# Franc-Z/CuClarabel

Hardware: AMD Instinct MI355X
Metric: KKT factorize+solve/sec (fp64) per IPM iter, 100k-var SOCP (higher is better)
Workload: dtype f64

## Files before the change

### cuclarabel_amd/csrc/factor_kernels.hip

```cpp
#include "kernels.hpp"
#include "knobs.hpp"
#include <utility>

namespace hipkkt {

__device__ inline double rl_f64(double v, int lane)
{
    const int lo = __builtin_amdgcn_readlane(__double2loint(v), lane);
    const int hi = __builtin_amdgcn_readlane(__double2hiint(v), lane);
    return __hiloint2double(hi, lo);
}
#define WAVE_FENCE() asm volatile("" ::: "memory")

__device__ __forceinline__ void lds_add(double* p, double v)
{
    __hip_atomic_fetch_add(p, v, __ATOMIC_RELAXED, __HIP_MEMORY_SCOPE_WORKGROUP);
}
#define OV_LD(p) __hip_atomic_load((p), __ATOMIC_RELAXED, __HIP_MEMORY_SCOPE_AGENT)
#define OV_ST(p, v) __hip_atomic_store((p), (v), __ATOMIC_RELAXED, __HIP_MEMORY_SCOPE_AGENT)
__device__ inline bool ov_wait_ge(const int* counter, int target, int* abort_word, long long t0, long long limit, int who = 0, int info = 0,
                                  int* seen_min = nullptr)
{
    for (;;) {
        const int seen = __hip_atomic_load(counter, __ATOMIC_RELAXED, __HIP_MEMORY_SCOPE_AGENT);
// ... 577 lines not shown
        }
        if (A.stamps) { long long t1 = wall_clock64(); t_iii += t1 - t0; }
    }
    __syncthreads();
    HIPKKT_STAMP(A, 4);
    if (!OV) for (int idx = tid; idx < f * nc; idx += BS) {
        const int j = idx / f, r = idx - j * f;
        if (!SLICED) {
            if (r >= j) F[idx] = P[r + pcol(j, f)];
        } else if (r >= nc) {
            F[(r_lo + r - nc) + (int64_t)j * ff] = P[r + pcol(j, f)];
        } else if (first && r >= j) {
            F[r + (int64_t)j * ff] = P[r + pcol(j, f)];
        }
    }
    __syncthreads();
    HIPKKT_STAMP(A, 5);
    if (A.stamps && blockIdx.x == 0 && tid == 0) {
        A.stamps[A.stamp_row * 16 + 8] = t_i;
        A.stamps[A.stamp_row * 16 + 9] = t_ii;
        A.stamps[A.stamp_row * 16 + 10] = t_iii;
        A.stamps[A.stamp_row * 16 + 11] = f;
        A.stamps[A.stamp_row * 16 + 12] = nc;
        A.stamps[A.stamp_row * 16 + 13] = T.child_ptr[s + 1] - T.child_ptr[s];
        A.stamps[A.stamp_row * 16 + 14] = clock64() - clk0;
    }
}

constexpr int TS = 64;
constexpr int KC = 16;

constexpr int LDA = TS + 16;

template <bool OV, bool PIPE>
__global__ __launch_bounds__(256) __attribute__((amdgpu_waves_per_eu(OV ? 3 : 4))) void k_schur(FactorArgs A, const int2* __restrict__ tiles, int tile_begin, int ntiles)
{
    __shared__ __attribute__((aligned(16))) double smem_s[TS * (TS + 1) + (OV ? 2 * KC * LDA + 2 : 0)];
    double (*As)[LDA] = reinterpret_cast<double (*)[LDA]>(smem_s + (OV ? TS * (TS + 1) : 0));
    double (*Bs)[LDA] = reinterpret_cast<double (*)[LDA]>(smem_s + (OV ? TS * (TS + 1) : 0) + KC * LDA);
    double (*Ct)[TS + 1] = reinterpret_cast<double (*)[TS + 1]>(smem_s);
    volatile int* sh_ok = reinterpret_cast<volatile int*>(smem_s + TS * (TS + 1) + 2 * KC * LDA);
    static_assert(2 * KC * LDA <= TS * (TS + 1), "operand chunks must fit under the tile buffer");
    const int tid = threadIdx.x, lane = tid & 63;
    const int wv = __builtin_amdgcn_readfirstlane(tid >> 6);
    const TreeDev& T = A.T;
    for (int tix = blockIdx.x; tix < ntiles; tix += gridDim.x) {
    const int2 tl = tiles[tile_begin + tix];
    const int s = tl.x;
    const int ti = tl.y >> 16, tj = tl.y & 0xffff;
    const int c0 = T.sn_start[s];
    const int nc = T.sn_start[s + 1] - c0;
    const int nb = (int)(T.rowptr[s + 1] - T.rowptr[s]);
    const int f = nc + nb;
    const double* __restrict__ F = A.fronts + T.front_off[s];
    double* __restrict__ U = A.upd + T.upd_off[s];
    const int r0 = ti * TS, q0 = tj * TS;
    const int nr = min(TS, nb - r0), nq = min(TS, nb - q0);

    const int wr = wv >> 1, wc = wv & 1;
    const bool active = !(ti == tj && wr < wc) && 32 * wr < nr && 32 * wc < nq;
    d4_t acc[2][2];
#pragma unroll
    for (int i = 0; i < 2; ++i)
#pragma unroll
        for (int j = 0; j < 2; ++j) acc[i][j] = (d4_t){0.0, 0.0, 0.0, 0.0};
    const int ml = lane & 15, mk = lane >> 4;
    const int64_t* __restrict__ tc = T.tile_cut + 5 * (int64_t)(tile_begin + tix);
    const int64_t i0 = tc[wv], i1 = tc[wv + 1];
    static_assert(sizeof(SubItem) == 16, "SubItem is read as an int4");
    const int4* __restrict__ sit4 = reinterpret_cast<const int4*>(T.sitems);
    int4 mine = (i0 < i1) ? sit4[min(i0 + lane, i1 - 1)] : make_int4(0, 0, 0, 0);
    auto pass_through = [&]() {
        constexpr int PT = 16;
        const int rlo = nc + r0;
        double* ct = &Ct[0][0];
        for (int64_t base = i0; base < i1; base += 64) {
            if (base > i0) mine = sit4[min(base + lane, i1 - 1)];
            const int n = (int)min((int64_t)64, i1 - base);
            for (int z0 = 0; z0 < n; z0 += PT) {
                double v[PT];
                int tg[PT];
#pragma unroll
                for (int z = 0; z < PT; ++z) {
                    const int src = min(z0 + z, 63);
                    const unsigned lo = (unsigned)__builtin_amdgcn_readlane(mine.x, src);
                    const int hi = __builtin_amdgcn_readlane(mine.y, src);
                    const int relstart = __builtin_amdgcn_readlane(mine.z, src);
                    const int cq = __builtin_amdgcn_readlane(mine.w, src);
                    const int64_t uoff = ((int64_t)hi << 32) | lo;
                    const int cnt = (z0 + z < n) ? (cq & 0xff) : 0, qcol = (cq >> 8) & 0xff;
                    const bool ok = lane < cnt;
                    v[z] = ok ? A.upd[uoff + lane] : 0.0;
                    tg[z] = ok ? qcol * (TS + 1) + (T.rel[relstart + lane] - rlo) : -1;
                }
#pragma unroll
                for (int z = 0; z < PT; ++z) if (tg[z] >= 0) lds_add(ct + tg[z], v[z]);
            }
        }
    };
    const int64_t dense_off_s = T.dense_off[s];
    auto dense_ptr = [&]() -> const double* {
        return dense_off_s >= 0 ? A.upd + dense_off_s + (int64_t)(nc + r0) + (int64_t)(nc + q0) * f : nullptr;
    };
    if (OV) {
        const double* __restrict__ Ud = dense_ptr();
        auto dense_at = [&](int a, int b) -> double {
            return (Ud && a < nr && b < nq && (r0 + a) >= (q0 + b)) ? Ud[a + (int64_t)b * f] : 0.0;
        };
// ... 176 lines not shown
void launch_front_wave(const FactorArgs& a, int begin, int count, int slice_doubles, hipStream_t st)
{
    if (count <= 0) return;
    init_factor_lds();
    hipLaunchKernelGGL(k_front_wave, dim3((count + 3) / 4), dim3(256), (size_t)4 * slice_doubles * sizeof(double), st,
                       a, begin, count, slice_doubles);
}
void launch_panel(const FactorArgs& a, int begin, int count, int bs, size_t lds, hipStream_t st)
{
    if (count <= 0) return;
    init_factor_lds();
    if (a.ov) {
        if (bs == 1024) hipLaunchKernelGGL((k_panel<1024, false, true>), dim3(count), dim3(1024), lds, st, a, begin);
        else if (bs == 512) hipLaunchKernelGGL((k_panel<512, false, true>), dim3(count), dim3(512), lds, st, a, begin);
        else hipLaunchKernelGGL((k_panel<256, false, true>), dim3(count), dim3(256), lds, st, a, begin);
        return;
    }
    if (bs == 1024) hipLaunchKernelGGL((k_panel<1024, false, false>), dim3(count), dim3(1024), lds, st, a, begin);
    else if (bs == 512) hipLaunchKernelGGL((k_panel<512, false, false>), dim3(count), dim3(512), lds, st, a, begin);
    else hipLaunchKernelGGL((k_panel<256, false, false>), dim3(count), dim3(256), lds, st, a, begin);
}
void launch_panel_sliced(const FactorArgs& a, int begin, int count, size_t lds, hipStream_t st)
{
    if (count <= 0) return;
    init_factor_lds();
    if (a.ov) hipLaunchKernelGGL((k_panel<1024, true, true>), dim3(count), dim3(1024), lds, st, a, begin);
    else hipLaunchKernelGGL((k_panel<1024, true, false>), dim3(count), dim3(1024), lds, st, a, begin);
}
void launch_schur(const FactorArgs& a, const int2* tiles, int tile_begin, int ntiles, hipStream_t st, int ov_grid, int tile_nc)
{
    if (ntiles <= 0) return;
    const int pipe_tiles = knobs().schur_pipe_tiles;
    const int pipe_nc = knobs().schur_pipe_nc;
    if (a.ov) hipLaunchKernelGGL((k_schur<true, true>), dim3(std::max(1, std::min(ntiles, ov_grid))), dim3(256), 0, st, a, tiles, tile_begin, ntiles);
    else if (ntiles > pipe_tiles && tile_nc >= pipe_nc) hipLaunchKernelGGL((k_schur<false, true>), dim3(ntiles), dim3(256), 0, st, a, tiles, tile_begin, ntiles);
    else hipLaunchKernelGGL((k_schur<false, false>), dim3(ntiles), dim3(256), 0, st, a, tiles, tile_begin, ntiles);
}

template <int VARIANT>
__global__ __launch_bounds__(256) void k_handover_litmus(double* payload, int* sig, int* ack, int words, int rounds,
                                                         unsigned long long* mismatches, unsigned long long* timeouts)
{
    __shared__ int sh_ok;
    const int pair = blockIdx.x >> 1, tid = threadIdx.x;
    const bool producer = (blockIdx.x & 1) == 0;
    double* pl = payload + (size_t)pair * words;
    const long long limit = 20000000;
    unsigned long long bad = 0;
    for (int r = 1; r <= rounds; ++r) {
        const long long t0 = wall_clock64();
        if (tid == 0) sh_ok = 1;
        __syncthreads();
        if (producer) {
            for (int w = tid; w < words; w += 256) {
                const double v = (double)r * 1024.0 + (double)w;
                if (VARIANT == 2) pl[w] = v; else OV_ST(pl + w, v);
            }
            if (VARIANT != 1) asm volatile("s_waitcnt vmcnt(0)" ::: "memory");
            __syncthreads();
            if (tid == 0) {
                OV_ST(sig + pair, r);
                for (;;) {
                    if (OV_LD(ack + pair) >= r) break;
                    if (wall_clock64() - t0 > limit) { sh_ok = 0; atomicAdd(timeouts, 1ull); break; }
                    __builtin_amdgcn_s_sleep(1);
                }
            }
            __syncthreads();
            if (!sh_ok) return;
// ... 31 lines not shown
```

### cuclarabel_amd/csrc/hipkkt.hip

```cpp
#include "../../include/hipkkt.h"

#include <hip/hip_runtime.h>

#include <algorithm>
#include <cfloat>
#include <chrono>
#include <cmath>
#include <cstdio>
#include <cstdlib>
#include <cstring>
#include <array>
#include <functional>
#include <map>
#include <memory>
#include <mutex>
#include <stdexcept>
#include <string>
#include <vector>

#include "kernels.hpp"
#include "kkt_assembly.hpp"
#include "symbolic.hpp"
#include "knobs.hpp"
#include "schedule.hpp"
#include "iterate_rows.hpp"

namespace hipkkt {

static thread_local std::string g_last_error;

struct ArgError : std::runtime_error { using std::runtime_error::runtime_error; };

#define HIP_CHECK(expr)                                                                          \
    do {                                                                                         \
        hipError_t e_ = (expr);                                                                  \
        if (e_ != hipSuccess)                                                                    \
            throw HipError(std::string(#expr) + ": " + hipGetErrorString(e_));                   \
    } while (0)

template <class T>
struct DBuf {
    T* p = nullptr;
    size_t n = 0;
    DBuf() = default;
    DBuf(const DBuf&) = delete;
    DBuf& operator=(const DBuf&) = delete;
    ~DBuf() { if (p) (void)hipFree(p); }
    void alloc(size_t count)
    {
        if (p) { (void)hipFree(p); p = nullptr; }
        n = count;
        HIP_CHECK(hipMalloc((void**)&p, std::max<size_t>(count, 1) * sizeof(T)));
    }
    void zero(hipStream_t st) { HIP_CHECK(hipMemsetAsync(p, 0, std::max<size_t>(n, 1) * sizeof(T), st)); }
    template <class V>
    void upload(const std::vector<V>& v)
    {
// ... 951 lines not shown
    {
        return knobs().factor_overlap;
    }
    bool ov_active() const { return overlap_wanted() && !ov_disabled && sch.ov_first < sch.launches.size(); }

    int* flags_ptr() { return flags.p; }

private:
    DBuf<int> d_sn_start, d_rows, d_rel, d_ncolpar, d_child_ptr, d_child_idx, d_ksrc, d_kdst, d_sched, d_perm;
    DBuf<int64_t> d_rowptr, d_front_off, d_upd_off, d_kptr;
    DBuf<signed char> d_psign;
    DBuf<double> fronts, upd, Dinv, xp, uvec, tinv;
    DBuf<double> xp_m, uvec_m;
    DBuf<int> d_iperm;
    size_t multi_cap = 0;
    DBuf<int64_t> d_tinv_off;
    DBuf<double> top_stamps;
    int n_stamp_sweeps = 0;
#ifdef HIPKKT_EXPERIMENTS
    int n_skipw_calls = 0;
#endif
    DBuf<int> d_tinv_list;
    DBuf<int> flags;
    DBuf<int64_t> stamps;
    DBuf<int64_t> d_tiles;
    DBuf<int64_t> d_cut_ptr;
    DBuf<int> d_cuts;
    DBuf<int64_t> d_item_ptr;
    DBuf<int64_t> d_items;
    DBuf<int64_t> d_dense_off;
    DBuf<int64_t> d_wave_cut;
    DBuf<int64_t> d_sitems;
    DBuf<int64_t> d_tile_cut;
    DBuf<int64_t> d_desc;
    DBuf<int64_t> d_sdesc;
    std::vector<int64_t> slice_kptr;
    std::vector<int> slice_nk;
    DBuf<int> d_spos, d_sn_parent, top_flags;
    DBuf<int> d_tk_pos, d_tk_sl, d_tbase;
    DBuf<double> xf;
    bool ov_disabled = false;
    bool ov_concurrent = false;
    DBuf<int> d_ov_prog, d_ov_done, d_ov_ntiles, d_ov_sprog, d_ov_sbase, d_ov_started;
    hipStream_t ov_stream = nullptr;
    hipEvent_t ev_ov_fork = nullptr, ev_ov_join = nullptr, ev_dev_done = nullptr;
    bool ov_join_pending = false;
    size_t nr_cap = 1;
    int top_epoch = 0;
    DBuf<int> d_gl_src, d_udst;
    DBuf<int64_t> d_glm_ptr, d_hp_lidx, d_pr_ptr;
    DBuf<int> d_udst_m, d_hp_col, d_hp_row, d_pr_slot;
    int n_pull_rows = 0;
    Schedule sch;
    DeviceLimits dev;
    NrGrids top_grid_nr;

    TreeDev tree() const
    {
        TreeDev t;
        t.nsuper = S.nsuper;
        t.sn_start = d_sn_start.p; t.rowptr = d_rowptr.p; t.rows = d_rows.p; t.rel = d_rel.p;
        t.ncolpar = d_ncolpar.p; t.front_off = d_front_off.p; t.upd_off = d_upd_off.p;
        t.child_ptr = d_child_ptr.p; t.child_idx = d_child_idx.p; t.kptr = d_kptr.p;
        t.ksrc = d_ksrc.p; t.kdst = d_kdst.p; t.sched = d_sched.p; t.psign = d_psign.p; t.perm = d_perm.p;
        t.dense_off = d_dense_off.p; t.item_ptr = d_item_ptr.p; t.items = (const ExtItem*)d_items.p; t.gl_ptr = d_item_ptr.p; t.gl_src = d_gl_src.p; t.udst = d_udst.p;
        t.glm_ptr = d_glm_ptr.p; t.udst_m = d_udst_m.p; t.hp_col = d_hp_col.p; t.hp_row = d_hp_row.p; t.hp_lidx = d_hp_lidx.p; t.pr_ptr = d_pr_ptr.p; t.pr_slot = d_pr_slot.p;
        t.cut_ptr = d_cut_ptr.p; t.cuts = d_cuts.p; t.wave_cut = d_wave_cut.p; t.tinv_off = d_tinv_off.p;
        t.sitems = (const SubItem*)d_sitems.p; t.tile_cut = d_tile_cut.p; t.desc = (const FrontDesc*)d_desc.p; t.sdesc = (const FrontDesc*)d_sdesc.p;
        t.spos = d_spos.p; t.sn_parent = d_sn_parent.p;
        return t;
    }

    int front_size(int s) const { return hipkkt::front_size(S, s); }

    void build_records(const std::vector<int64_t>& glptr, const std::vector<int>& gsrc)
    {
        if (sch.rec_refused_bytes && knobs().verbose)
            std::fprintf(stderr, "[hipkkt] packed sweep records would take %.0f MB: legacy layout\n", sch.rec_refused_bytes / 1048576.0);
        const int64_t total = sch.rec_bytes;
        if (total <= 0) return;
        std::vector<int64_t> store((size_t)(total / 8) + 8, 0);
        char* base = reinterpret_cast<char*>(store.data());
        for (size_t q = 0; q < sch.launches.size(); ++q) {
            const Launch& L = sch.launches[q];
            const bool leaf = rec_no_slots(sch.launches, q);
            RecClass classes[2];
            const int nclasses = rec_classes(L, classes);
            for (int ci = 0; ci < nclasses; ++ci) {
                const RecClass& c = classes[ci];
                const int fmax = L.rec.fmax[c.cls];
                for (int k = 0; k < c.count; ++k) {
                    const int sn = sch.sched[(size_t)(c.first + k)];
                    char* rec = base + L.rec.off[c.cls] + (int64_t)k * L.rec.stride[c.cls];
                    const int nc = S.sn_start[sn + 1] - S.sn_start[sn], nb = (int)(S.rowptr[sn + 1] - S.rowptr[sn]), f = nc + nb;
                    if (f > fmax) throw std::runtime_error("packed record: front larger than its class");
                    SolveHdr h{};
                    h.mat_off = c.cls == 0 ? h_toff[(size_t)sn] : S.front_off[sn];
                    h.rp = S.rowptr[sn];
                    h.s = sn; h.c0 = S.sn_start[sn]; h.nc = nc; h.nb = nb;
                    h.par = S.sn_parent[sn];
                    h.nchild = sch.nch.empty() ? 0 : sch.nch[(size_t)sn];
// ... 202 lines not shown
            std::vector<int> gsrc((size_t)ptr[nloc]);
            {
                std::vector<int64_t> nxt(ptr.begin(), ptr.end() - 1);
                for (int p = 0; p < S.nsuper; ++p)
                    for (int e = S.child_ptr[p]; e < S.child_ptr[p + 1]; ++e) {
                        int c = S.child_idx[e];
                        for (int64_t q = S.rowptr[c]; q < S.rowptr[c + 1]; ++q) gsrc[nxt[lbase(p) + S.rel[q]]++] = (int)q;
                    }
            }
            if (S.rows.size() >= ((size_t)1 << 31)) throw std::runtime_error("row structure exceeds int32 indexing");
            if (knobs().verbose >= 2 && sch.top_launches > 0) {
                long hist[6] = {0, 0, 0, 0, 0, 0};
                long fronts_over8 = 0, fronts_over12 = 0, nf = 0;
                int64_t gmax = 0;
                for (size_t q = sch.launches.size() - sch.top_launches; q < sch.launches.size(); ++q)
                    for (int t = sch.launches[q].begin; t < sch.launches[q].begin + sch.launches[q].count; ++t) {
                        const int sn = sch.sched[(size_t)t];
                        const int f = front_size(sn);
                        int64_t fm = 0;
                        for (int i = 0; i < f; ++i) {
                            const int64_t n = ptr[lbase(sn) + i + 1] - ptr[lbase(sn) + i];
                            hist[n == 0 ? 0 : n <= 4 ? 1 : n <= 8 ? 2 : n <= 12 ? 3 : n <= 16 ? 4 : 5]++;
                            fm = std::max(fm, n);
                        }
                        gmax = std::max(gmax, fm);
                        fronts_over8 += fm > 8; fronts_over12 += fm > 12; ++nf;
                    }
                std::fprintf(stderr, "[hipkkt] persistent solve set: gather sources per row: 0: %ld, 1-4: %ld, 5-8: %ld, 9-12: %ld, "
                             "13-16: %ld, more: %ld (max %lld); fronts with a row over 8: %ld, over 12: %ld of %ld\n",
                             hist[0], hist[1], hist[2], hist[3], hist[4], hist[5], (long long)gmax, fronts_over8, fronts_over12, nf);
            }
            d_item_ptr.upload(ptr);
            static_assert(sizeof(ExtItem) == 32, "ExtItem layout");
            std::vector<int> dense_child((size_t)S.nsuper, -1);
            std::vector<int64_t> dense_off((size_t)S.nsuper, -1);
            const bool dense_on = knobs().dense_child;
            int64_t n_dense = 0;
            for (int p = 0; dense_on && p < S.nsuper; ++p) {
                if (sch.tile_base[p] < 0) continue;
                const int fp = front_size(p);
                for (int e = S.child_ptr[p]; e < S.child_ptr[p + 1]; ++e) {
                    const int c = S.child_idx[e];
                    const int nbc = (int)(S.rowptr[c + 1] - S.rowptr[c]);
                    if (nbc != fp) continue;
                    bool ident = true;
                    for (int q = 0; ident && q < nbc; ++q) ident = S.rel[S.rowptr[c] + q] == q;
                    if (!ident) continue;
                    dense_child[(size_t)p] = c;
                    dense_off[(size_t)p] = S.upd_off[c];
                    ++n_dense;
                    break;
                }
            }
            d_dense_off.upload(dense_off);
            if (knobs().verbose) std::fprintf(stderr, "[hipkkt] dense children: %lld\n", (long long)n_dense);
            std::vector<int64_t> pptr((size_t)S.N + 1, 0);
            for (int c = 0; c < S.nsuper; ++c) {
                int p = S.sn_parent[c];
                if (p < 0 || dense_child[(size_t)p] == c) continue;
                const int pnc = S.sn_start[p + 1] - S.sn_start[p];
                const int nbc = (int)(S.rowptr[c + 1] - S.rowptr[c]);
                for (int b = 0; b < nbc; ++b) {
                    const int r = S.rel[S.rowptr[c] + b];
                    if (r >= pnc) break;
                    pptr[(size_t)S.sn_start[p] + r + 1] += (nbc - b + 63) / 64;
                }
            }
            for (int i = 0; i < S.N; ++i) pptr[i + 1] += pptr[i];
            std::vector<ExtItem> items((size_t)pptr[S.N]);
            {
                std::vector<int64_t> nxt(pptr.begin(), pptr.end() - 1);
                for (int p = 0; p < S.nsuper; ++p) {
                    const int pnc = S.sn_start[p + 1] - S.sn_start[p];
                    for (int e = S.child_ptr[p]; e < S.child_ptr[p + 1]; ++e) {
                        int c = S.child_idx[e];
                        if (dense_child[(size_t)p] == c) continue;
                        int nbc = (int)(S.rowptr[c + 1] - S.rowptr[c]);
                        for (int b = 0; b < nbc; ++b) {
                            int64_t q = S.rowptr[c] + b;
                            const int r = S.rel[q];
                            if (r >= pnc) break;
                            for (int a = b; a < nbc; a += 64) {
                                ExtItem it;
                                it.uoff = S.upd_off[c] + (int64_t)b * nbc + a;
                                it.relstart = (int)(S.rowptr[c] + a);
                                it.cnt = std::min(64, nbc - a);
// ... 34 lines not shown
                        if (e.rfirst >= nc && (e.rlast < r_lo || e.rfirst >= r_lo + rs)) continue;
                        items.push_back(e);
                    }
                }
                scp[(size_t)nc] = (int64_t)items.size();
                const int64_t I0 = scp[0], I1 = scp[(size_t)nc];
                int j = 0;
                int64_t* w = wcut.data() + ((size_t)S.nsuper + q) * 17;
                for (int k = 0; k < 16; ++k) {
                    const int64_t target = I0 + ((I1 - I0) * k) / 16;
                    while (j < nc && scp[(size_t)j] < target) ++j;
                    w[k] = scp[(size_t)j];
                }
                w[16] = I1;
            }
            std::vector<int64_t> raw(std::max<size_t>(items.size(), 1) * 4);
            std::memcpy(raw.data(), items.data(), items.size() * sizeof(ExtItem));
            d_items.upload(raw);
            d_wave_cut.upload(wcut);
            if (knobs().verbose) {
                if (knobs().verbose >= 2) {
                    for (size_t q = sch.sched.size() > 12 ? sch.sched.size() - 12 : 0; q < sch.sched.size(); ++q) {
                        const int sn = sch.sched[q];
                        const int64_t* w = wcut.data() + (size_t)sn * 17;
                        int64_t mx = 0, rows = 0;
                        for (int k = 0; k < 16; ++k) mx = std::max(mx, w[k + 1] - w[k]);
                        for (int64_t it = w[0]; it < w[16]; ++it) rows += items[(size_t)it].cnt;
                        std::fprintf(stderr, "[hipkkt] front %d f %d nc %d kids %d: %lld panel items (%lld entries), largest wave slice %lld\n",
                                     sn, front_size(sn), S.sn_start[sn + 1] - S.sn_start[sn], S.child_ptr[sn + 1] - S.child_ptr[sn],
                                     (long long)(w[16] - w[0]), (long long)rows, (long long)mx);
                    }
                }
            }
            static_assert(sizeof(SubItem) == 16, "SubItem layout");
            const int64_t ntile = (int64_t)sch.tiles.size();
            std::vector<int64_t> cnt((size_t)ntile * 64 + 1, 0);
            auto for_each_sub = [&](auto&& fn) {
                for (int p = 0; p < S.nsuper; ++p) {
                    if (sch.tile_base[p] < 0) continue;
                    const int pnc = S.sn_start[p + 1] - S.sn_start[p];
                    for (int e = S.child_ptr[p]; e < S.child_ptr[p + 1]; ++e) {
                        const int c = S.child_idx[e];
                        if (dense_child[(size_t)p] == c) continue;
                        const int nbc = (int)(S.rowptr[c + 1] - S.rowptr[c]);
                        const int* rl = S.rel.data() + S.rowptr[c];
                        for (int b = 0; b < nbc; ++b) {
                            if (rl[b] < pnc) continue;
                            const int j = rl[b] - pnc, tj = j >> 6;
                            int a = b;
                            while (a < nbc) {
                                const int ti = (rl[a] - pnc) >> 6;
                                int a2 = a;
                                while (a2 < nbc && ((rl[a2] - pnc) >> 6) == ti) ++a2;
                                const int64_t tile = sch.tile_base[p] + (int64_t)ti * (ti + 1) / 2 + tj;
                                fn(tile, j & 63, c, b, a, a2 - a, nbc);
                                a = a2;
                            }
                        }
                    }
                }
            };
            for_each_sub([&](int64_t tile, int q, int, int, int, int, int) { cnt[tile * 64 + q + 1]++; });
            for (size_t i = 0; i + 1 < cnt.size(); ++i) cnt[i + 1] += cnt[i];
            std::vector<SubItem> sit((size_t)cnt.back());
            {
                std::vector<int64_t> nx(cnt.begin(), cnt.end() - 1);
                for_each_sub([&](int64_t tile, int q, int c, int b, int a, int n, int nbc) {
                    SubItem si;
                    si.uoff = S.upd_off[c] + (int64_t)b * nbc + a;
                    si.relstart = (int)(S.rowptr[c] + a);
                    si.cnt = (unsigned char)n;
                    si.qcol = (unsigned char)q;
                    si.pad = 0;
                    sit[(size_t)nx[tile * 64 + q]++] = si;
                });
            }
            std::vector<int64_t> tcut((size_t)ntile * 5 + 5, 0);
            for (int64_t t = 0; t < ntile; ++t) {
                const int64_t* cp = cnt.data() + t * 64;
                const int64_t I0 = cp[0], I1 = cp[64];
                int q = 0;
                for (int w = 0; w < 4; ++w) {
                    const int64_t target = I0 + ((I1 - I0) * w) / 4;
                    while (q < 64 && cp[q] < target) ++q;
                    tcut[t * 5 + w] = cp[q];
                }
                tcut[t * 5 + 4] = I1;
            }
            std::vector<int64_t> tiles_up(sch.tiles);
            {
                const int tile_xcd = knobs().tile_xcd;
                if (tile_xcd > 0) {
                    std::vector<int64_t> nc2(tcut);
                    for (const Launch& L : sch.launches) {
                        if (L.small || L.count < tile_xcd || L.ntiles <= 0) continue;
                        std::vector<std::pair<int64_t, int64_t>> rng;
                        for (int t = L.begin; t < L.begin + L.count; ++t) {
                            const int sn = sch.sched[(size_t)t];
                            if (sch.tile_base[sn] < 0) continue;
                            const int nb = front_size(sn) - (S.sn_start[sn + 1] - S.sn_start[sn]);
                            const int k = (nb + 63) / 64;
                            if (k > 0) rng.push_back({sch.tile_base[sn], sch.tile_base[sn] + (int64_t)k * (k + 1) / 2});
                        }
                        int64_t pos = L.tile_begin;
                        for (size_t g0 = 0; g0 < rng.size(); g0 += 8) {
                            const size_t g1 = std::min(rng.size(), g0 + 8);
                            int64_t longest = 0;
                            for (size_t x = g0; x < g1; ++x) longest = std::max(longest, rng[x].second - rng[x].first);
                            for (int64_t j = 0; j < longest; ++j)
                                for (size_t x = g0; x < g1; ++x)
                                    if (rng[x].first + j < rng[x].second) {
                                        const int64_t from = rng[x].first + j;
                                        tiles_up[(size_t)pos] = sch.tiles[(size_t)from];
                                        for (int w = 0; w < 5; ++w) nc2[(size_t)pos * 5 + w] = tcut[(size_t)from * 5 + w];
                                        ++pos;
                                    }
                        }
                        if (pos != (int64_t)L.tile_begin + L.ntiles) throw std::runtime_error("tile permutation lost a tile");
                    }
                    tcut.swap(nc2);
                }
            }
            d_tiles.upload(tiles_up);
            std::vector<int64_t> raw2(sit.size() * 2);
            std::memcpy(raw2.data(), sit.data(), sit.size() * sizeof(SubItem));
            d_sitems.upload(raw2);
            d_tile_cut.upload(tcut);
            d_gl_src.upload(gsrc);
            build_records(ptr, gsrc);
            std::vector<int> ud(std::max<size_t>(S.rows.size(), 1), 0);
            for (size_t g = 0; g < gsrc.size(); ++g) ud[(size_t)gsrc[g]] = (int)g;
            d_udst.upload(ud);
            {
                std::vector<int> row_sn(std::max<size_t>(S.rows.size(), 1), -1);
                for (int c = 0; c < S.nsuper; ++c)
                    for (int64_t q = S.rowptr[c]; q < S.rowptr[c + 1]; ++q) row_sn[(size_t)q] = c;
                std::vector<int64_t> mptr((size_t)nloc + 1, 0), prp(1, 0);
                std::vector<int> udm(std::max<size_t>(S.rows.size(), 1), -1), hcol, prs;
                std::vector<int64_t> hl;
                int64_t slot = 0;
                for (int64_t lc = 0; lc < nloc; ++lc) {
                    mptr[(size_t)lc] = slot;
                    bool any = false;
                    for (int64_t g = ptr[(size_t)lc]; g < ptr[(size_t)lc + 1] && !any; ++g) any = pulled[(size_t)row_sn[(size_t)gsrc[(size_t)g]]] != 0;
                    if (any) prs.push_back((int)slot++);
                    for (int64_t g = ptr[(size_t)lc]; g < ptr[(size_t)lc + 1]; ++g) {
                        const int q = gsrc[(size_t)g], c = row_sn[(size_t)q];
                        if (pulled[(size_t)c]) {
                            hcol.push_back(S.sn_start[c]);
                            hl.push_back(S.front_off[c] + 1 + ((int64_t)q - S.rowptr[c]));
                        } else {
                            udm[(size_t)q] = (int)slot++;
                        }
                    }
                    if (any) prp.push_back((int64_t)hcol.size());
                }
                mptr[(size_t)nloc] = slot;
                n_pull_rows = (int)prs.size();
                if (hcol.empty()) { hcol.push_back(0); hl.push_back(0); }
                if (prs.empty()) prs.push_back(0);
// ... 2566 lines not shown
```

### cuclarabel_amd/csrc/kernels.hpp

```cpp
#pragma once
#include <hip/hip_runtime.h>
#include "launch_shapes.hpp"
#include <cstdint>
#include <mutex>
#include <stdexcept>
#include <string>

namespace hipkkt {

struct HipError : std::runtime_error { using std::runtime_error::runtime_error; };

class PerDeviceOnce {
    std::mutex mu_;
    uint64_t done_[4] = {0, 0, 0, 0};
public:
    template <class F>
    void run(F&& fn)
    {
        int dev = 0;
        if (hipGetDevice(&dev) != hipSuccess || dev < 0 || dev >= 256) throw HipError("hipGetDevice failed");
        std::lock_guard<std::mutex> lk(mu_);
        if (done_[dev >> 6] >> (dev & 63) & 1) return;
        const hipError_t e = fn();
        if (e != hipSuccess) {
// ... 60 lines not shown
    const int64_t* front_off;
    const int64_t* upd_off;
    const int* child_ptr;
    const int* child_idx;
    const int64_t* kptr;
    const int* ksrc;
    const int* kdst;
    const int* sched;
    const int* spos;
    const int* sn_parent;
    const FrontDesc* sdesc;
    const FrontDesc* desc;
    const signed char* psign;
    const int* perm;
    const int64_t* item_ptr;
    const ExtItem* items;
    const int64_t* dense_off;
    const int64_t* gl_ptr;
    const int* gl_src;
    const int* udst;
    const int64_t* glm_ptr;
    const int* udst_m;
    const int* hp_col;
    const int* hp_row;
    const int64_t* hp_lidx;
    const int64_t* pr_ptr;
    const int* pr_slot;
    const int64_t* cut_ptr;
    const int* cuts;
    const int64_t* wave_cut;
    const int64_t* tinv_off;
    const SubItem* sitems;
    const int64_t* tile_cut;
};

struct FactorArgs {
    TreeDev T;
    const double* Kval;
    const double* eps;
    double* fronts;
    double* upd;
    double* Dinv;
    int* flags;
    int* ov_prog;
    int* ov_done;
    const int* ov_ntiles;
    int* ov_sprog;
    const int* ov_sbase;
    int* ov_started;
    int ov_slot;
    int ov;
    long long ov_limit;
    double dyn_eps, dyn_delta;
    int nbk;
    long long* stamps;
    int stamp_row;
};
#define HIPKKT_STAMP(A, k) do { if ((A).stamps && blockIdx.x == 0 && threadIdx.x == 0) \
        (A).stamps[(A).stamp_row * 16 + (k)] = wall_clock64(); } while (0)

struct SolveArgs {
    TreeDev T;
    const double* fronts;
    const double* tinv;
    const double* Dinv;
    const double* b;
// ... 285 lines not shown
```

### cuclarabel_amd/csrc/knobs.hpp

```cpp
#pragma once
#include <cstdlib>

namespace hipkkt {

#define HIPKKT_KNOBS(KNOB, FLAG_SET, FLAG_ON)                                                                                         \
                                                                                                                 \
    KNOB(int, verbose, "HIPKKT_VERBOSE", 0)                  \
    FLAG_SET(stamps, "HIPKKT_STAMPS")                                    \
    KNOB(int, top_stamps, "HIPKKT_TOP_STAMPS", 0)            \
    KNOB(int, top_stamps_nr, "HIPKKT_TOP_STAMPS_NR", 1)                                       \
    FLAG_SET(dump_levels, "HIPKKT_DUMP_LEVELS")                                \
    FLAG_SET(dump_subtrees, "HIPKKT_DUMP_SUBTREES")                        \
                                                                                      \
    KNOB(double, nd_sep_ratio, "HIPKKT_ND_SEP_RATIO", 0.10)  \
    KNOB(int, nd_sep_min, "HIPKKT_ND_SEP_MIN", 5000)                                           \
    KNOB(long long, panel_cap, "HIPKKT_PANEL_CAP", -1)       \
    KNOB(int, panel_max_cols, "HIPKKT_PANEL_MAX_COLS", -1)                                                  \
    KNOB(int, panel_slice_below, "HIPKKT_PANEL_SLICE_BELOW", -1)  \
    FLAG_SET(postorder_layout, "HIPKKT_POSTORDER_LAYOUT")                       \
    FLAG_ON(upd_pingpong, "HIPKKT_UPD_PINGPONG")                                        \
    KNOB(int, bundle_kids, "HIPKKT_BUNDLE_KIDS", 200)        \
    KNOB(int, bundle_kids_panel, "HIPKKT_BUNDLE_KIDS_PANEL", 400)   \
    FLAG_ON(bundle_cost, "HIPKKT_BUNDLE_COST")               \
                                                                                                  \
    KNOB(int, merge_small, "HIPKKT_MERGE_SMALL", 128)        \
    KNOB(int, slice_rows, "HIPKKT_SLICE_ROWS", 128)            \
    FLAG_ON(slice_fit, "HIPKKT_SLICE_FIT")                                    \
    KNOB(int, bs128_count, "HIPKKT_BS128_COUNT", 1024)                                 \
    KNOB(int, bs128_f, "HIPKKT_BS128_F", 128)                         \
    KNOB(int, solve_tall_rows, "HIPKKT_SOLVE_TALL_ROWS", 0)  \
    KNOB(int, tall_block_rows, "HIPKKT_TALL_BLOCK_ROWS", 256)  \
    FLAG_ON(dense_child, "HIPKKT_DENSE_CHILD")               \
    KNOB(int, tile_xcd, "HIPKKT_TILE_XCD", 150)              \
    FLAG_ON(pull_leaves, "HIPKKT_PULL_LEAVES")                   \
    FLAG_ON(packed, "HIPKKT_PACKED")                            \
    KNOB(long long, packed_max_mb, "HIPKKT_PACKED_MAX_MB", 4096)                       \
                                                                                                               \
    FLAG_SET(graph, "HIPKKT_GRAPH")                               \
    FLAG_SET(no_overlap, "HIPKKT_NO_OVERLAP")                                                         \
    KNOB(int, winv_tail, "HIPKKT_WINV_TAIL", 4)                \
    KNOB(int, winv_early, "HIPKKT_WINV_EARLY", 1)                                                   \
    KNOB(int, winv_blocks, "HIPKKT_WINV_BLOCKS", 0)                           \
    FLAG_ON(winv_split, "HIPKKT_WINV_SPLIT")                 \
    FLAG_ON(winv_run_forks, "HIPKKT_WINV_RUN_FORKS")                        \
    FLAG_ON(factor_overlap, "HIPKKT_FACTOR_OVERLAP")                 \
    FLAG_SET(ov_cu_mask, "HIPKKT_OV_CU_MASK")                                        \
    KNOB(long long, ov_test_limit, "HIPKKT_OV_TEST_LIMIT", 5000000)   \
    KNOB(int, ov_max_fronts, "HIPKKT_OV_MAX_FRONTS", 0)      \
    KNOB(int, ov_max_tiles, "HIPKKT_OV_MAX_TILES", 1600)     \
    KNOB(int, ov_merge, "HIPKKT_OV_MERGE", 100)                   \
    KNOB(int, ov_merge_wide, "HIPKKT_OV_MERGE_WIDE", 24)                     \
    KNOB(int, ov_merge_groups, "HIPKKT_OV_MERGE_GROUPS", 8)                                \
    KNOB(int, schur_pipe_tiles, "HIPKKT_SCHUR_PIPE_TILES", 1600)                     \
    KNOB(int, schur_pipe_nc, "HIPKKT_SCHUR_PIPE_NC", 64)            \
                                                                                                                      \
    FLAG_SET(no_top, "HIPKKT_NO_TOP")                                                            \
    KNOB(int, top_tall, "HIPKKT_TOP_TALL", -1)                                        \
    KNOB(int, top_cap, "HIPKKT_TOP_CAP", 1 << 30)                                        \
    KNOB(double, top_mult, "HIPKKT_TOP_MULT", 1.5)                            \
    KNOB(long long, top_test_limit, "HIPKKT_TOP_TEST_LIMIT", 5000000)  \
    FLAG_SET(no_level_merge, "HIPKKT_NO_LEVEL_MERGE")               \
    KNOB(int, solve_slice_kb, "HIPKKT_SOLVE_SLICE_KB", 80)                                  \
    KNOB(int, solve_slice_max, "HIPKKT_SOLVE_SLICE_MAX", 64)                                     \
    KNOB(long long, solve_slice_from, "HIPKKT_SOLVE_SLICE_FROM", -1)  \
    FLAG_ON(chain, "HIPKKT_CHAIN")                                                           \
    FLAG_ON(chain_top, "HIPKKT_CHAIN_TOP")                   \
    KNOB(int, chain_max, "HIPKKT_CHAIN_MAX", 640)                                             \
    FLAG_SET(test_publish_fail, "HIPKKT_TEST_PUBLISH_FAIL")  \
    KNOB(int, multi_vec, "HIPKKT_MULTI_VEC", 4)                                    \
    KNOB(int, multi_ct, "HIPKKT_MULTI_CT", 0)

struct Knobs {
#define HIPKKT_K_FIELD(type, field, name, dflt) type field = dflt;
#define HIPKKT_K_FLAG(field, name) bool field = false;
#define HIPKKT_K_FLAGON(field, name) bool field = true;
    HIPKKT_KNOBS(HIPKKT_K_FIELD, HIPKKT_K_FLAG, HIPKKT_K_FLAGON)
#undef HIPKKT_K_FIELD
#undef HIPKKT_K_FLAG
#undef HIPKKT_K_FLAGON
    static void get(int& v, const char* e) { v = std::atoi(e); }
    static void get(long long& v, const char* e) { v = std::atoll(e); }
    static void get(double& v, const char* e) { v = std::atof(e); }
    Knobs()
    {
#define HIPKKT_K_READ(type, field, name, dflt) if (const char* e_ = std::getenv(name)) get(field, e_);
#define HIPKKT_K_READF(field, name) field = std::getenv(name) != nullptr;
#define HIPKKT_K_READON(field, name) if (const char* e_ = std::getenv(name)) field = std::atoi(e_) != 0;
// ... 15 lines not shown
```

Baseline: 318.5.

## Pack short Schur scatter pieces into merged slots with precomputed targets

Adds a host-side builder that merges short child-update pieces (at most the threshold entries) within each wave into packed slots holding per-entry source-offset/target records. The pass-through kernel gains a packed variant that reads these records, so a single readlane slot covers up to 64 entries instead of one short piece, and it prefetches the next batch's records ahead of the LDS atomic adds. This cuts the number of serialized slot iterations and the wasted lanes for small pieces. In exchange it adds an extra indirection array, more preprocessing, and a fallback to the legacy lists when the packed stream exceeds a size cap.

```diff
diff --git a/cuclarabel_amd/csrc/factor_kernels.hip b/cuclarabel_amd/csrc/factor_kernels.hip
--- a/cuclarabel_amd/csrc/factor_kernels.hip
+++ b/cuclarabel_amd/csrc/factor_kernels.hip
@@ -633,7 +633,7 @@
 
 constexpr int LDA = TS + 16;
 
-template <bool OV, bool PIPE>
+template <bool OV, bool PIPE, bool PK>
 __global__ __launch_bounds__(256) __attribute__((amdgpu_waves_per_eu(OV ? 3 : 4))) void k_schur(FactorArgs A, const int2* __restrict__ tiles, int tile_begin, int ntiles)
 {
     __shared__ __attribute__((aligned(16))) double smem_s[TS * (TS + 1) + (OV ? 2 * KC * LDA + 2 : 0)];
@@ -675,6 +675,55 @@
         constexpr int PT = 16;
         const int rlo = nc + r0;
         double* ct = &Ct[0][0];
+        if (PK) {
+            const unsigned* __restrict__ recs = T.slot_recs;
+            const unsigned* __restrict__ relw = reinterpret_cast<const unsigned*>(T.rel);
+            const int nbatch = (int)((i1 - i0 + PT - 1) / PT);
+            unsigned w[PT];
+            int4 cur = mine;
+            auto stage_a = [&](const int4& hd, int k) {
+                const int z0 = (k & 3) * PT;
+                const int n = (int)min((int64_t)64, i1 - (i0 + (int64_t)(k >> 2) * 64));
+#pragma unroll
+                for (int z = 0; z < PT; ++z) {
+                    const int src = z0 + z;
+                    const int aux = __builtin_amdgcn_readlane(hd.z, src);
+                    const int cq = __builtin_amdgcn_readlane(hd.w, src);
+                    const int cnt = (src < n) ? (cq & 0xff) : 0;
+                    const unsigned* p = ((cq >> 16) & 1) ? recs + aux : relw + aux;
+                    w[z] = (lane < cnt) ? p[lane] : 0u;
+                }
+            };
+            if (nbatch > 0) stage_a(cur, 0);
+            for (int k = 0; k < nbatch; ++k) {
+                double v[PT];
+                int tg[PT];
+                const int z0 = (k & 3) * PT;
+                const int n = (int)min((int64_t)64, i1 - (i0 + (int64_t)(k >> 2) * 64));
+#pragma unroll
+                for (int z = 0; z < PT; ++z) {
+                    const int src = z0 + z;
+                    const unsigned lo = (unsigned)__builtin_amdgcn_readlane(cur.x, src);
+                    const int hi = __builtin_amdgcn_readlane(cur.y, src);
+                    const int cq = __builtin_amdgcn_readlane(cur.w, src);
+                    const int64_t uoff = ((int64_t)hi << 32) | lo;
+                    const int cnt = (src < n) ? (cq & 0xff) : 0, qcol = (cq >> 8) & 0xff;
+                    const bool pk = ((cq >> 16) & 1) != 0;
+                    const bool ok = lane < cnt;
+                    const int d = pk ? (int)(w[z] >> 13) : lane;
+                    const int t = pk ? (int)(w[z] & 8191u) : qcol * (TS + 1) + ((int)w[z] - rlo);
+                    v[z] = ok ? A.upd[uoff + d] : 0.0;
+                    tg[z] = ok ? t : -1;
+                }
+                int4 nxt = cur;
+                if (((k + 1) & 3) == 0 && k + 1 < nbatch) nxt = sit4[min(i0 + (int64_t)(k + 1) * PT + lane, i1 - 1)];
+                stage_a(nxt, k + 1);
+#pragma unroll
+                for (int z = 0; z < PT; ++z) if (tg[z] >= 0) lds_add(ct + tg[z], v[z]);
+                cur = nxt;
+            }
+            return;
+        }
         for (int64_t base = i0; base < i1; base += 64) {
             if (base > i0) mine = sit4[min(base + lane, i1 - 1)];
             const int n = (int)min((int64_t)64, i1 - base);
@@ -917,9 +966,12 @@
     if (ntiles <= 0) return;
     const int pipe_tiles = knobs().schur_pipe_tiles;
     const int pipe_nc = knobs().schur_pipe_nc;
-    if (a.ov) hipLaunchKernelGGL((k_schur<true, true>), dim3(std::max(1, std::min(ntiles, ov_grid))), dim3(256), 0, st, a, tiles, tile_begin, ntiles);
-    else if (ntiles > pipe_tiles && tile_nc >= pipe_nc) hipLaunchKernelGGL((k_schur<false, true>), dim3(ntiles), dim3(256), 0, st, a, tiles, tile_begin, ntiles);
-    else hipLaunchKernelGGL((k_schur<false, false>), dim3(ntiles), dim3(256), 0, st, a, tiles, tile_begin, ntiles);
+    const bool pk = a.T.slot_recs != nullptr;
+    const dim3 grid(a.ov ? std::max(1, std::min(ntiles, ov_grid)) : ntiles);
+    auto go = [&](auto kernel) { hipLaunchKernelGGL(kernel, grid, dim3(256), 0, st, a, tiles, tile_begin, ntiles); };
+    if (a.ov) pk ? go(k_schur<true, true, true>) : go(k_schur<true, true, false>);
+    else if (ntiles > pipe_tiles && tile_nc >= pipe_nc) pk ? go(k_schur<false, true, true>) : go(k_schur<false, true, false>);
+    else pk ? go(k_schur<false, false, true>) : go(k_schur<false, false, false>);
 }
 
 template <int VARIANT>
diff --git a/cuclarabel_amd/csrc/hipkkt.hip b/cuclarabel_amd/csrc/hipkkt.hip
--- a/cuclarabel_amd/csrc/hipkkt.hip
+++ b/cuclarabel_amd/csrc/hipkkt.hip
@@ -23,6 +23,7 @@
 #include "symbolic.hpp"
 #include "knobs.hpp"
 #include "schedule.hpp"
+#include "schur_stream.hpp"
 #include "iterate_rows.hpp"
 
 namespace hipkkt {
@@ -1040,6 +1041,8 @@
     DBuf<int64_t> d_wave_cut;
     DBuf<int64_t> d_sitems;
     DBuf<int64_t> d_tile_cut;
+    DBuf<unsigned> d_slot_recs;
+    bool schur_packed = false;
     DBuf<int64_t> d_desc;
     DBuf<int64_t> d_sdesc;
     std::vector<int64_t> slice_kptr;
@@ -1074,7 +1077,7 @@
         t.dense_off = d_dense_off.p; t.item_ptr = d_item_ptr.p; t.items = (const ExtItem*)d_items.p; t.gl_ptr = d_item_ptr.p; t.gl_src = d_gl_src.p; t.udst = d_udst.p;
         t.glm_ptr = d_glm_ptr.p; t.udst_m = d_udst_m.p; t.hp_col = d_hp_col.p; t.hp_row = d_hp_row.p; t.hp_lidx = d_hp_lidx.p; t.pr_ptr = d_pr_ptr.p; t.pr_slot = d_pr_slot.p;
         t.cut_ptr = d_cut_ptr.p; t.cuts = d_cuts.p; t.wave_cut = d_wave_cut.p; t.tinv_off = d_tinv_off.p;
-        t.sitems = (const SubItem*)d_sitems.p; t.tile_cut = d_tile_cut.p; t.desc = (const FrontDesc*)d_desc.p; t.sdesc = (const FrontDesc*)d_sdesc.p;
+        t.sitems = (const SubItem*)d_sitems.p; t.tile_cut = d_tile_cut.p; t.slot_recs = schur_packed ? d_slot_recs.p : nullptr; t.desc = (const FrontDesc*)d_desc.p; t.sdesc = (const FrontDesc*)d_sdesc.p;
         t.spos = d_spos.p; t.sn_parent = d_sn_parent.p;
         return t;
     }
@@ -1343,26 +1346,11 @@
             }
             d_item_ptr.upload(ptr);
             static_assert(sizeof(ExtItem) == 32, "ExtItem layout");
-            std::vector<int> dense_child((size_t)S.nsuper, -1);
+            const std::vector<int> dense_child = find_dense_children(S, sch.tile_base, knobs().dense_child);
             std::vector<int64_t> dense_off((size_t)S.nsuper, -1);
-            const bool dense_on = knobs().dense_child;
             int64_t n_dense = 0;
-            for (int p = 0; dense_on && p < S.nsuper; ++p) {
-                if (sch.tile_base[p] < 0) continue;
-                const int fp = front_size(p);
-                for (int e = S.child_ptr[p]; e < S.child_ptr[p + 1]; ++e) {
-                    const int c = S.child_idx[e];
-                    const int nbc = (int)(S.rowptr[c + 1] - S.rowptr[c]);
-                    if (nbc != fp) continue;
-                    bool ident = true;
-                    for (int q = 0; ident && q < nbc; ++q) ident = S.rel[S.rowptr[c] + q] == q;
-                    if (!ident) continue;
-                    dense_child[(size_t)p] = c;
-                    dense_off[(size_t)p] = S.upd_off[c];
-                    ++n_dense;
-                    break;
-                }
-            }
+            for (int p = 0; p < S.nsuper; ++p)
+                if (dense_child[(size_t)p] >= 0) { dense_off[(size_t)p] = S.upd_off[dense_child[(size_t)p]]; ++n_dense; }
             d_dense_off.upload(dense_off);
             if (knobs().verbose) std::fprintf(stderr, "[hipkkt] dense children: %lld\n", (long long)n_dense);
             std::vector<int64_t> pptr((size_t)S.N + 1, 0);
@@ -1463,61 +1451,34 @@
                     }
                 }
             }
-            static_assert(sizeof(SubItem) == 16, "SubItem layout");
+            static_assert(sizeof(SubItem) == sizeof(SchurSlot), "SubItem is the image of SchurSlot");
             const int64_t ntile = (int64_t)sch.tiles.size();
-            std::vector<int64_t> cnt((size_t)ntile * 64 + 1, 0);
-            auto for_each_sub = [&](auto&& fn) {
-                for (int p = 0; p < S.nsuper; ++p) {
-                    if (sch.tile_base[p] < 0) continue;
-                    const int pnc = S.sn_start[p + 1] - S.sn_start[p];
-                    for (int e = S.child_ptr[p]; e < S.child_ptr[p + 1]; ++e) {
-                        const int c = S.child_idx[e];
-                        if (dense_child[(size_t)p] == c) continue;
-                        const int nbc = (int)(S.rowptr[c + 1] - S.rowptr[c]);
-                        const int* rl = S.rel.data() + S.rowptr[c];
-                        for (int b = 0; b < nbc; ++b) {
-                            if (rl[b] < pnc) continue;
-                            const int j = rl[b] - pnc, tj = j >> 6;
-                            int a = b;
-                            while (a < nbc) {
-                                const int ti = (rl[a] - pnc) >> 6;
-                                int a2 = a;
-                                while (a2 < nbc && ((rl[a2] - pnc) >> 6) == ti) ++a2;
-                                const int64_t tile = sch.tile_base[p] + (int64_t)ti * (ti + 1) / 2 + tj;
-                                fn(tile, j & 63, c, b, a, a2 - a, nbc);
-                                a = a2;
-                            }
-                        }
+            SchurStreamOptions sso;
+            sso.pack = knobs().schur_pack;
+            sso.threshold = std::min(64, std::max(1, knobs().schur_pack_max));
+            sso.max_bytes = (int64_t)knobs().packed_max_mb << 20;
+            SchurStream sst = build_schur_stream(S, sch.tile_base, ntile, dense_child, sso);
+            schur_packed = sst.packed;
+            if (knobs().verbose) {
+                if (sst.refused_bytes) std::fprintf(stderr, "[hipkkt] packed Schur stream would take %.0f MB: legacy lists\n", sst.refused_bytes / 1048576.0);
+                for (const Launch& L : sch.launches) {
+                    if (L.small || L.ntiles <= 0) continue;
+                    long long pieces = 0, entries = 0, slots = 0, r0 = 0, r1 = 0, recs = 0;
+                    for (int64_t t = L.tile_begin; t < (int64_t)L.tile_begin + L.ntiles; ++t) {
+                        pieces += sst.pieces[(size_t)t]; entries += sst.entries[(size_t)t];
+                        slots += sst.cut[(size_t)t * 5 + 4] - sst.cut[(size_t)t * 5];
+                        int64_t wmax = 0;
+                        for (int w = 0; w < 4; ++w) wmax = std::max(wmax, sst.cut[(size_t)t * 5 + w + 1] - sst.cut[(size_t)t * 5 + w]);
+                        r0 += (sst.legacy_wave_max[(size_t)t] + 15) / 16; r1 += (wmax + 15) / 16;
+                        for (int64_t i = sst.cut[(size_t)t * 5]; i < sst.cut[(size_t)t * 5 + 4]; ++i)
+                            if (sst.slots[(size_t)i].packed) recs += sst.slots[(size_t)i].cnt;
                     }
+                    std::fprintf(stderr, "[hipkkt] schur stream level %d: %d tiles, %lld pieces of %.1f entries, slots %lld -> %lld, load rounds per tile "
+                                 "%.2f -> %.2f, %lld bytes\n", L.level, L.ntiles, pieces, pieces ? (double)entries / pieces : 0.0, pieces, slots,
+                                 (double)r0 / L.ntiles, (double)r1 / L.ntiles, slots * 16 + recs * 4);
                 }
-            };
-            for_each_sub([&](int64_t tile, int q, int, int, int, int, int) { cnt[tile * 64 + q + 1]++; });
-            for (size_t i = 0; i + 1 < cnt.size(); ++i) cnt[i + 1] += cnt[i];
-            std::vector<SubItem> sit((size_t)cnt.back());
-            {
-                std::vector<int64_t> nx(cnt.begin(), cnt.end() - 1);
-                for_each_sub([&](int64_t tile, int q, int c, int b, int a, int n, int nbc) {
-                    SubItem si;
-                    si.uoff = S.upd_off[c] + (int64_t)b * nbc + a;
-                    si.relstart = (int)(S.rowptr[c] + a);
-                    si.cnt = (unsigned char)n;
-                    si.qcol = (unsigned char)q;
-                    si.pad = 0;
-                    sit[(size_t)nx[tile * 64 + q]++] = si;
-                });
-            }
-            std::vector<int64_t> tcut((size_t)ntile * 5 + 5, 0);
-            for (int64_t t = 0; t < ntile; ++t) {
-                const int64_t* cp = cnt.data() + t * 64;
-                const int64_t I0 = cp[0], I1 = cp[64];
-                int q = 0;
-                for (int w = 0; w < 4; ++w) {
-                    const int64_t target = I0 + ((I1 - I0) * w) / 4;
-                    while (q < 64 && cp[q] < target) ++q;
-                    tcut[t * 5 + w] = cp[q];
-                }
-                tcut[t * 5 + 4] = I1;
-            }
+            }
+            std::vector<int64_t>& tcut = sst.cut;
             std::vector<int64_t> tiles_up(sch.tiles);
             {
                 const int tile_xcd = knobs().tile_xcd;
@@ -1553,10 +1514,14 @@
                 }
             }
             d_tiles.upload(tiles_up);
-            std::vector<int64_t> raw2(sit.size() * 2);
-            std::memcpy(raw2.data(), sit.data(), sit.size() * sizeof(SubItem));
+            std::vector<int64_t> raw2(sst.slots.size() * 2);
+            std::memcpy(raw2.data(), sst.slots.data(), sst.slots.size() * sizeof(SchurSlot));
             d_sitems.upload(raw2);
             d_tile_cut.upload(tcut);
+            if (sst.packed) {
+                if (sst.recs.empty()) sst.recs.push_back(0);
+                d_slot_recs.upload(sst.recs);
+            }
             d_gl_src.upload(gsrc);
             build_records(ptr, gsrc);
             std::vector<int> ud(std::max<size_t>(S.rows.size(), 1), 0);
diff --git a/cuclarabel_amd/csrc/kernels.hpp b/cuclarabel_amd/csrc/kernels.hpp
--- a/cuclarabel_amd/csrc/kernels.hpp
+++ b/cuclarabel_amd/csrc/kernels.hpp
@@ -116,6 +116,7 @@
     const int64_t* tinv_off;
     const SubItem* sitems;
     const int64_t* tile_cut;
+    const unsigned* slot_recs;
 };
 
 struct FactorArgs {
diff --git a/cuclarabel_amd/csrc/knobs.hpp b/cuclarabel_amd/csrc/knobs.hpp
--- a/cuclarabel_amd/csrc/knobs.hpp
+++ b/cuclarabel_amd/csrc/knobs.hpp
@@ -53,6 +53,8 @@
     KNOB(int, ov_merge_groups, "HIPKKT_OV_MERGE_GROUPS", 8)                                \
     KNOB(int, schur_pipe_tiles, "HIPKKT_SCHUR_PIPE_TILES", 1600)                     \
     KNOB(int, schur_pipe_nc, "HIPKKT_SCHUR_PIPE_NC", 64)            \
+    FLAG_ON(schur_pack, "HIPKKT_SCHUR_PACK")                 \
+    KNOB(int, schur_pack_max, "HIPKKT_SCHUR_PACK_MAX", 32)                         \
                                                                                                                       \
     FLAG_SET(no_top, "HIPKKT_NO_TOP")                                                            \
     KNOB(int, top_tall, "HIPKKT_TOP_TALL", -1)                                        \
diff --git a/cuclarabel_amd/csrc/schur_stream.cpp b/cuclarabel_amd/csrc/schur_stream.cpp
--- /dev/null
+++ b/cuclarabel_amd/csrc/schur_stream.cpp
@@ -0,0 +1,220 @@
+#include "schur_stream.hpp"
+
+#include <algorithm>
+#include <stdexcept>
+
+namespace hipkkt {
+
+namespace {
+
+struct Piece {
+    int64_t uoff;
+    int relstart;
+    int rlo;
+    unsigned char cnt, qcol;
+};
+
+struct WavePacker {
+    const Symbolic& S;
+    SchurStream& R;
+    const int threshold;
+    std::vector<int> last = std::vector<int>((size_t)64 * kSchurTileLd, -1);
+    std::vector<int> touched;
+    size_t first_slot = 0;
+    int open_idx = -1, open_pieces = 0;
+    Piece open_first{};
+    std::vector<int64_t> osrc;
+    std::vector<int> otgt;
+    int64_t omin = 0, omax = 0;
+
+    WavePacker(const Symbolic& s, SchurStream& r, int thr) : S(s), R(r), threshold(thr) {}
+
+    int target(const Piece& p, int k) const { return p.qcol * kSchurTileLd + (S.rel[(size_t)p.relstart + k] - p.rlo); }
+    static SchurSlot long_slot(const Piece& p)
+    {
+        SchurSlot s;
+        s.base = p.uoff; s.aux = p.relstart; s.cnt = p.cnt; s.qcol = p.qcol; s.packed = 0;
+        return s;
+    }
+    void touch(int tgt, int idx)
+    {
+        if (last[(size_t)tgt] < 0) touched.push_back(tgt);
+        last[(size_t)tgt] = idx;
+    }
+    void close()
+    {
+        if (open_idx < 0) return;
+        SchurSlot& s = R.slots[first_slot + (size_t)open_idx];
+        if (open_pieces == 1) {
+            s = long_slot(open_first);
+        } else {
+            s.base = omin; s.aux = (int)R.recs.size(); s.cnt = (unsigned char)osrc.size(); s.qcol = 0; s.packed = 1;
+            for (size_t k = 0; k < osrc.size(); ++k)
+                R.recs.push_back((uint32_t)(osrc[k] - omin) << kSchurTgtBits | (uint32_t)otgt[k]);
+        }
+        open_idx = -1; open_pieces = 0;
+        osrc.clear(); otgt.clear();
+    }
+    void add(const Piece& p)
+    {
+        if (p.cnt > threshold) {
+            const int idx = (int)(R.slots.size() - first_slot);
+            R.slots.push_back(long_slot(p));
+            for (int k = 0; k < p.cnt; ++k) touch(target(p, k), idx);
+            return;
+        }
+        const int64_t lo = p.uoff, hi = p.uoff + p.cnt - 1;
+        bool join = open_idx >= 0 && osrc.size() + p.cnt <= 64 && std::max(omax, hi) - std::min(omin, lo) < kSchurMaxDelta;
+        for (int k = 0; join && k < p.cnt; ++k) join = last[(size_t)target(p, k)] < open_idx;
+        if (!join) {
+            close();
+            open_idx = (int)(R.slots.size() - first_slot);
+            R.slots.push_back(SchurSlot{});
+            open_first = p;
+            omin = lo; omax = hi;
+        }
+        omin = std::min(omin, lo); omax = std::max(omax, hi);
+        ++open_pieces;
+        for (int k = 0; k < p.cnt; ++k) {
+            const int tgt = target(p, k);
+            osrc.push_back(p.uoff + k);
+            otgt.push_back(tgt);
+            touch(tgt, open_idx);
+        }
+    }
+    void begin() { first_slot = R.slots.size(); }
+    void end()
+    {
+        close();
+        for (int t : touched) last[(size_t)t] = -1;
+        touched.clear();
+    }
+};
+
+}
+
+std::vector<int> find_dense_children(const Symbolic& S, const std::vector<int64_t>& tile_base, bool on)
+{
+    std::vector<int> dense_child((size_t)S.nsuper, -1);
+    for (int p = 0; on && p < S.nsuper; ++p) {
+        if (tile_base[(size_t)p] < 0) continue;
+        const int fp = (S.sn_start[p + 1] - S.sn_start[p]) + (int)(S.rowptr[p + 1] - S.rowptr[p]);
+        for (int e = S.child_ptr[p]; e < S.child_ptr[p + 1]; ++e) {
+            const int c = S.child_idx[e];
+            const int nbc = (int)(S.rowptr[c + 1] - S.rowptr[c]);
+            if (nbc != fp) continue;
+            bool ident = true;
+            for (int q = 0; ident && q < nbc; ++q) ident = S.rel[(size_t)S.rowptr[c] + q] == q;
+            if (!ident) continue;
+            dense_child[(size_t)p] = c;
+            break;
+        }
+    }
+    return dense_child;
+}
+
+SchurStream build_schur_stream(const Symbolic& S, const std::vector<int64_t>& tile_base, int64_t ntile,
+                               const std::vector<int>& dense_child, const SchurStreamOptions& opt)
+{
+    if (opt.threshold < 1 || opt.threshold > 64) throw std::runtime_error("Schur stream: packing threshold outside 1..64");
+    SchurStream R;
+    auto for_each_piece = [&](auto&& fn) {
+        for (int p = 0; p < S.nsuper; ++p) {
+            if (tile_base[(size_t)p] < 0) continue;
+            const int pnc = S.sn_start[p + 1] - S.sn_start[p];
+            for (int e = S.child_ptr[p]; e < S.child_ptr[p + 1]; ++e) {
+                const int c = S.child_idx[e];
+                if (dense_child[(size_t)p] == c) continue;
+                const int nbc = (int)(S.rowptr[c + 1] - S.rowptr[c]);
+                const int* rl = S.rel.data() + S.rowptr[c];
+                for (int b = 0; b < nbc; ++b) {
+                    if (rl[b] < pnc) continue;
+                    const int j = rl[b] - pnc, tj = j >> 6;
+                    int a = b;
+                    while (a < nbc) {
+                        const int ti = (rl[a] - pnc) >> 6;
+                        int a2 = a;
+                        while (a2 < nbc && ((rl[a2] - pnc) >> 6) == ti) ++a2;
+                        const int64_t tile = tile_base[(size_t)p] + (int64_t)ti * (ti + 1) / 2 + tj;
+                        Piece pc;
+                        pc.uoff = S.upd_off[c] + (int64_t)b * nbc + a;
+                        pc.relstart = (int)(S.rowptr[c] + a);
+                        pc.rlo = pnc + ti * 64;
+                        pc.cnt = (unsigned char)(a2 - a);
+                        pc.qcol = (unsigned char)(j & 63);
+                        fn(tile, pc);
+                        a = a2;
+                    }
+                }
+            }
+        }
+    };
+    std::vector<int64_t> cnt((size_t)ntile * 64 + 1, 0);
+    R.pieces.assign((size_t)ntile, 0);
+    R.entries.assign((size_t)ntile, 0);
+    R.legacy_wave_max.assign((size_t)ntile, 0);
+    for_each_piece([&](int64_t tile, const Piece& pc) {
+        cnt[(size_t)tile * 64 + pc.qcol + 1]++;
+        R.pieces[(size_t)tile]++;
+        R.entries[(size_t)tile] += pc.cnt;
+    });
+    for (size_t i = 0; i + 1 < cnt.size(); ++i) cnt[i + 1] += cnt[i];
+    std::vector<int64_t> tcut((size_t)ntile * 5 + 5, 0);
+    for (int64_t t = 0; t < ntile; ++t) {
+        const int64_t* cp = cnt.data() + t * 64;
+        const int64_t I0 = cp[0], I1 = cp[64];
+        int q = 0;
+        for (int w = 0; w < 4; ++w) {
+            const int64_t target = I0 + ((I1 - I0) * w) / 4;
+            while (q < 64 && cp[q] < target) ++q;
+            tcut[(size_t)t * 5 + w] = cp[q];
+        }
+        tcut[(size_t)t * 5 + 4] = I1;
+        for (int w = 0; w < 4; ++w)
+            R.legacy_wave_max[(size_t)t] = std::max(R.legacy_wave_max[(size_t)t], (int)(tcut[(size_t)t * 5 + w + 1] - tcut[(size_t)t * 5 + w]));
+    }
+    const size_t npiece = (size_t)cnt.back();
+    if (!opt.pack) {
+        R.slots.resize(npiece);
+        std::vector<int64_t> nx(cnt.begin(), cnt.end() - 1);
+        for_each_piece([&](int64_t tile, const Piece& pc) { R.slots[(size_t)nx[(size_t)tile * 64 + pc.qcol]++] = WavePacker::long_slot(pc); });
+        R.cut.swap(tcut);
+        return R;
+    }
+    std::vector<Piece> pcs(npiece);
+    {
+        std::vector<int64_t> nx((size_t)ntile * 4);
+        for (int64_t t = 0; t < ntile; ++t)
+            for (int w = 0; w < 4; ++w) nx[(size_t)t * 4 + w] = tcut[(size_t)t * 5 + w];
+        for_each_piece([&](int64_t tile, const Piece& pc) {
+            const int64_t at = cnt[(size_t)tile * 64 + pc.qcol];
+            const int64_t* tc = tcut.data() + tile * 5;
+            int w = 0;
+            while (w < 3 && at >= tc[w + 1]) ++w;
+            pcs[(size_t)nx[(size_t)tile * 4 + w]++] = pc;
+        });
+    }
+    R.packed = true;
+    R.cut.assign((size_t)ntile * 5 + 5, 0);
+    WavePacker pk(S, R, opt.threshold);
+    for (int64_t t = 0; t < ntile; ++t) {
+        for (int w = 0; w < 4; ++w) {
+            R.cut[(size_t)t * 5 + w] = (int64_t)R.slots.size();
+            pk.begin();
+            for (int64_t i = tcut[(size_t)t * 5 + w]; i < tcut[(size_t)t * 5 + w + 1]; ++i) pk.add(pcs[(size_t)i]);
+            pk.end();
+        }
+        R.cut[(size_t)t * 5 + 4] = (int64_t)R.slots.size();
+    }
+    for (size_t i = (size_t)ntile * 5; i < R.cut.size(); ++i) R.cut[i] = (int64_t)R.slots.size();
+    if (R.bytes() > opt.max_bytes || R.recs.size() >= ((size_t)1 << 31)) {
+        const int64_t refused = R.bytes();
+        SchurStreamOptions legacy = opt;
+        legacy.pack = false;
+        R = build_schur_stream(S, tile_base, ntile, dense_child, legacy);
+        R.refused_bytes = refused;
+    }
+    return R;
+}
+
+}
diff --git a/cuclarabel_amd/csrc/schur_stream.hpp b/cuclarabel_amd/csrc/schur_stream.hpp
--- /dev/null
+++ b/cuclarabel_amd/csrc/schur_stream.hpp
@@ -0,0 +1,43 @@
+#pragma once
+#include <cstdint>
+#include <vector>
+
+#include "symbolic.hpp"
+
+namespace hipkkt {
+
+struct SchurSlot {
+    int64_t base;
+    int aux;
+    unsigned char cnt;
+    unsigned char qcol;
+    unsigned short packed;
+};
+static_assert(sizeof(SchurSlot) == 16, "SchurSlot layout");
+
+constexpr int kSchurTgtBits = 13;
+constexpr int kSchurTileLd = 65;
+constexpr int64_t kSchurMaxDelta = (int64_t)1 << (32 - kSchurTgtBits);
+
+struct SchurStreamOptions {
+    bool pack = true;
+    int threshold = 32;
+    int64_t max_bytes = (int64_t)4096 << 20;
+};
+
+struct SchurStream {
+    bool packed = false;
+    std::vector<SchurSlot> slots;
+    std::vector<uint32_t> recs;
+    std::vector<int64_t> cut;
+    int64_t refused_bytes = 0;
+    std::vector<int> pieces, entries, legacy_wave_max;
+    int64_t bytes() const { return (int64_t)slots.size() * 16 + (int64_t)recs.size() * 4; }
+};
+
+std::vector<int> find_dense_children(const Symbolic& S, const std::vector<int64_t>& tile_base, bool on);
+
+SchurStream build_schur_stream(const Symbolic& S, const std::vector<int64_t>& tile_base, int64_t ntile,
+                               const std::vector<int>& dense_child, const SchurStreamOptions& opt);
+
+}
```

Result: no change. 316.3 (-0.7%).
